# TUMFTM/global_racetrajectory_optimization

Measured on NVIDIA H100. Metric: min-curv QPs/sec (N=1000 closed track, batched), higher is better.
Workload: dtype f64

## Files before the change

global_racetrajectory_optimization_b200/csrc/mincurv_ipm.cu:

```cuda
#include <cstdio>
#include <cstdlib>
#include "capi.cuh"
#include "mincurv_ops.cuh"

namespace mc {

constexpr unsigned FULL = 0xffffffffu;
constexpr int IP_THREADS = 64;
constexpr int SUB = 8;
constexpr int VBP = 12;
constexpr int FROW = 33;
constexpr int HB_SLOTS = 2;
constexpr int HO_SLOTS = 2;
constexpr int LROW = 33;
#ifndef MC_LT_SLOTS
#define MC_LT_SLOTS 3
#endif
constexpr int LT_SLOTS = MC_LT_SLOTS;
constexpr int GT_SLOTS = 6 - LT_SLOTS;
constexpr int RING_UNITS = LT_SLOTS + GT_SLOTS;
constexpr int QDEPTH = 16;
constexpr int LT_UNIT_DOUBLES = SUB * LROW;
constexpr int GT_UNIT_DOUBLES = SUB * FROW;
constexpr unsigned HB_UNIT_BYTES = SUB * HB_PITCH * sizeof(double);
// ... 644 lines not shown
    sh.gs[lane] = gsl - (s0 + s1);
}

__device__ __noinline__ void sweep_sep_solve(IpShared &sh, double *__restrict__ GTp, const double *Zp, const int NA, double *__restrict__ x) {
    const int lane = threadIdx.x & 31;
    const int nunits = (NA + SUB - 1) / SUB;
    GtRing R(sh, &sh.u.sw.gt[0][0], GTp, nunits, true);
    R.prime();
    double a = sh.gs[lane];
#pragma unroll 4
    for (int k = 0; k < 32; ++k) {
        const double yk = __shfl_sync(FULL, a, k);
        const double l = (lane > k) ? sh.s.Ss[lane * 33 + k] : 0.0;
        a = fma(-l, yk, a);
    }
    a *= sh.wS[lane];
#pragma unroll 4
    for (int k = 31; k >= 0; --k) {
        const double xk = __shfl_sync(FULL, a, k);
        const double l = (lane < k) ? sh.s.Ss[k * 33 + lane] : 0.0;
        a = fma(-l, xk, a);
    }
    x[NA + lane] = a;
    const int kl = lane & 7, qr = lane >> 3;
    double xq[8];
#pragma unroll
    for (int i = 0; i < 8; ++i) xq[i] = __shfl_sync(FULL, a, 8 * qr + i);
    double znext = 0.0;
    if (nunits > 0 && R.unit(0) * SUB + kl < NA) znext = Zp[R.unit(0) * SUB + kl];
    for (int i = 0; i < nunits; ++i, R.next()) {
        const int k = R.unit(i) * SUB + kl;
        const double z = znext;
        if (i + 1 < nunits && R.unit(i + 1) * SUB + kl < NA) znext = Zp[R.unit(i + 1) * SUB + kl];
        if ((i & 7) == 0 && i >= 8) prog_wait<true>(sh, &sh.prog[2], i - 8);
        const double *gt = R.wait() + kl * FROW;
        double c0 = 0.0, c1 = 0.0;
#pragma unroll
        for (int e = 0; e < 8; e += 2) {
            c0 = fma(gt[8 * qr + e], xq[e], c0);
            c1 = fma(gt[8 * qr + e + 1], xq[e + 1], c1);
        }
        double c = c0 + c1;
        c += __shfl_xor_sync(FULL, c, 8);
        c += __shfl_xor_sync(FULL, c, 16);
        if (qr == 0) sh.u.sw.q[(i & (QDEPTH - 1)) * SUB + kl] = (k < NA) ? fma(-c, gt[32], z) : 0.0;
        __syncwarp();
        if (lane == 0) { prog_publish(&sh.prog[3], i + 1); R.refill(i); }
    }
    R.close();
}

__device__ __noinline__ void sweep_backward(IpShared &sh, double *__restrict__ LTp, const int NA, double *__restrict__ x) {
    const int lane = threadIdx.x & 31;
    const int gq = lane >> 2, q = lane & 3;
    const int nunits = (NA + SUB - 1) / SUB;
    LtRing R(sh, &sh.u.sw.lt[0][0], LTp, nunits, true);
    R.prime();
    double nbx[8];
#pragma unroll
    for (int i = 0; i < 8; ++i) nbx[i] = 0.0;
    for (int i = 0; i < nunits; ++i, R.next()) {
        const int k0 = R.unit(i) * SUB;
        const double *lt = R.wait();
        double a[10];
#pragma unroll
        for (int c = 0; c < 10; ++c) a[c] = lt_entry(lt, gq, 4 * c + q);
        double c0[2] = {0.0, 0.0}, c1[2] = {0.0, 0.0};
#pragma unroll
        for (int e = 2; e < 8; e += 2) {
            dmma(c0, a[2 + e], nbx[e]);
            dmma(c1, a[3 + e], nbx[e + 1]);
        }
        dmma(c0, a[2], nbx[0]);
        dmma(c1, a[3], nbx[1]);
        prog_wait(sh, &sh.prog[3], i + 1);
        const double t1 = sh.u.sw.q[(i & (QDEPTH - 1)) * SUB + gq];
        const double uu = t1 + (c0[0] + c1[0]);
        const double u0 = __shfl_sync(FULL, uu, 4 * q), u1 = __shfl_sync(FULL, uu, 16 + 4 * q);
        double d0[2] = {uu, uu}, d1[2] = {0.0, 0.0};
        dmma(d0, a[0], u0);
        dmma(d1, a[1], u1);
        const double x1 = d0[0] + d1[0];
        if (q == 0 && k0 + gq < NA) x[k0 + gq] = x1;
#pragma unroll
        for (int e = 7; e >= 2; --e) nbx[e] = nbx[e - 2];
        nbx[0] = -__shfl_sync(FULL, x1, 4 * q);
        nbx[1] = -__shfl_sync(FULL, x1, 16 + 4 * q);
        __syncwarp();
        if (lane == 0) { prog_publish(&sh.prog[2], i + 1); R.refill(i); }
    }
    R.close();
}

__device__ __noinline__ void solve(IpShared &sh, double *slab, const Layout &L, int n, const double *g, double *x, bool fused) {
    const Factor F = make_factor(slab, L, n, nullptr);
    const int warp = threadIdx.x >> 5;
    if (threadIdx.x < 4) sh.prog[threadIdx.x] = 0;
    fence_proxy_async();
    __syncthreads();
    if (!fused) {
        PROF_T0(t0);
        if (warp == 0) sweep_forward(sh, F.LT, F.Z, F.NA, g);
        else sweep_sep_rhs(sh, F.GT, F.NA, g);
        __syncthreads();
        PROF_ADD1(PROF_FWD_SWEEPS, t0);
    }
    PROF_T0(t3);
    if (warp == 1) sweep_sep_solve(sh, F.GT, F.Z, F.NA, x);
    else sweep_backward(sh, F.LT, F.NA, x);
    __syncthreads();
    PROF_ADD1(PROF_BWD_SWEEPS, t3);
}

__device__ void band_matvec(const double *__restrict__ HB, const double *__restrict__ v, double *__restrict__ out, int n) {
    for (int i = threadIdx.x; i < n; i += IP_THREADS) {
        const double *row = HB + (size_t)i * HB_PITCH;
        double s = row[0] * v[i];
        int j = i;
        for (int k = 1; k <= HBW; ++k) {
            j = (j + 1 == n) ? 0 : j + 1;
            s = fma(row[k], v[j], s);
        }
        j = i;
        for (int k = 1; k <= HBW; ++k) {
            j = (j == 0) ? n - 1 : j - 1;
            s = fma(HB[(size_t)j * HB_PITCH + k], v[j], s);
        }
        out[i] = s;
    }
}

__device__ __forceinline__ IpShared &ip_init_shared() {
    extern __shared__ __align__(16) unsigned char smem_raw[];
    IpShared &sh = *reinterpret_cast<IpShared *>(smem_raw);
    if (threadIdx.x == 0) {
        for (int i = 0; i < HB_SLOTS; ++i) mbar_init(&sh.hb_full[i], 1);
        for (int i = 0; i < HO_SLOTS; ++i) { mbar_init(&sh.ho_full[i], 1); mbar_init(&sh.ho_empty[i], 1); }
        for (int i = 0; i < RING_UNITS; ++i) mbar_init(&sh.ring_full[i], 1);
        sh.ring_phase[0] = 0; sh.ring_phase[1] = 0;
        asm volatile("fence.mbarrier_init.release.cluster;" ::: "memory");
    }
    __syncthreads();
    return sh;
}

__device__ __forceinline__ int next_instance(IpShared &sh, int *work_counter) {
    __syncthreads();
    if (threadIdx.x == 0) sh.next = atomicAdd(work_counter, 1);
    __syncthreads();
    return sh.next;
}

constexpr int V_PARK = V_VV;
enum ParkSlot {
    PARK_MU = 0, PARK_MU0 = 1, PARK_RDTOL = 2, PARK_IT = 3,
    PARK_TRACE = 8,
    PARK_MU_HIST = 16,
    PARK_LIST = 64
};
constexpr int PARK_BUCKETS = 24;
enum SchedSlot { SCHED_WORK = 0, SCHED_COUNT = 8, SCHED_TAKEN = 40 };
static_assert(SCHED_WORK < SCHED_COUNT && SCHED_COUNT + PARK_BUCKETS <= SCHED_TAKEN && SCHED_TAKEN + PARK_BUCKETS <= SCHED_INTS,
              "the schedule's counters behind the slabs");
static_assert(PARK_MU_HIST + 40 <= PARK_LIST && PARK_LIST + PARK_BUCKETS / 2 <= N_MIN + 64, "V_PARK slots within a vector");

__device__ __forceinline__ double *park_slots(double *ws, const Layout &L, int b) { return vec(ws + (size_t)b * L.stride, L, V_PARK); }
__device__ __forceinline__ int *park_list(double *ws, const Layout &L, int r) { return reinterpret_cast<int *>(park_slots(ws, L, r) + PARK_LIST); }
__device__ __forceinline__ int ld_relaxed(const int *p) {
    int v;
    asm volatile("ld.relaxed.gpu.global.s32 %0, [%1];" : "=r"(v) : "l"(p) : "memory");
    return v;
}

__device__ __forceinline__ int park_bucket(double mu, double mu_prev, double target, int left, int n, int n_max) {
    double r = left;
    if (mu <= target) r = 1.0;
    else if (mu < mu_prev) r = ceil(log(target / mu) / log(mu / mu_prev)) + 1.0;
    r = fmin(fmax(r, 1.0), (double)left);
    return min(PARK_BUCKETS - 1, (int)ceil(r * n / n_max));
}

__device__ __forceinline__ void park(int *sched, double *ws, const Layout &L, int b, int k) {
    __threadfence();
    const int r = atomicAdd(&sched[SCHED_COUNT + k], 1);
    atomicExch(&park_list(ws, L, r)[k], b + 1);
}

__device__ __forceinline__ int next_work(IpShared &sh, int *sched, double *ws, const Layout &L, int B) {
    __syncthreads();
    if (threadIdx.x == 0) {
        int b = B, resumed = 0;
        if (ld_relaxed(&sched[SCHED_WORK]) < B) b = atomicAdd(&sched[SCHED_WORK], 1);
        if (b >= B) {
            b = B;
            for (int k = PARK_BUCKETS - 1; k >= 0 && !resumed; --k) {
                int t = ld_relaxed(&sched[SCHED_TAKEN + k]);
                while (t < ld_relaxed(&sched[SCHED_COUNT + k])) {
                    const int seen = atomicCAS(&sched[SCHED_TAKEN + k], t, t + 1);
                    if (seen != t) { t = seen; continue; }
                    const int *e = &park_list(ws, L, t)[k];
                    int v = 0;
                    for (int spin = 0; spin < (1 << 24) && (v = ld_relaxed(e)) == 0; ++spin) __nanosleep(64);
                    __threadfence();
                    if (v > 0) { b = v - 1; resumed = 1; }
                    break;
                }
            }
        }
        sh.next = b;
        sh.resumed = resumed;
    }
    __syncthreads();
    return sh.next;
}

#ifdef MC_TAIL_TRACE
__device__ __forceinline__ double trace_clock() {
    unsigned long long t;
    asm volatile("mov.u64 %0, %%globaltimer;" : "=l"(t));
    return __longlong_as_double((long long)t);
}
#endif

template <bool ADD_ITERS>
__device__ __forceinline__ void write_instance(double *aout, int n, int n_max, const double *AL, int b, int result, int it,
                                               int32_t *status, int32_t *iters_out) {
    __syncthreads();
    for (int i = threadIdx.x; i < n_max; i += IP_THREADS) aout[i] = (i < n) ? AL[i] : 0.0;
    if (threadIdx.x == 0) {
        status[b] = result;
        if (iters_out) iters_out[b] = ADD_ITERS ? iters_out[b] + it : it;
    }
}

__device__ __forceinline__ double affine_step(double r) { return (r > 1.0) ? 1.0 / r : 1.0; }
__device__ __forceinline__ double centring(double c00, double c01, double c10, double c11, double ap, double ad, double mu, double m) {
    const double sigma = (c00 + ad * c01 + ap * c10 + ap * ad * c11) / m / mu;
    return sigma * sigma * sigma * mu;
}
__device__ __forceinline__ double damped_step(double eta, double r) { return (eta < r) ? eta / r : 1.0; }
__device__ __forceinline__ void corrector_terms(double smu, double su, double sl, double lu, double ll, double dx, double isu,
                                                double isl, double &tu, double &tl) {
    const double dlu = lu * (dx * isu - 1.0), dll = -ll * (1.0 + dx * isl);
    tu = smu - su * lu + dx * dlu;
    tl = smu - sl * ll - dx * dll;
}

__global__ void __launch_bounds__(IP_THREADS, 8)
mincurv_pdip_kernel(int B, int n_max, const int32_t *__restrict__ n_pts, double *__restrict__ ws, Layout L,
                    PdipParams prm, int slice, double *__restrict__ alpha_out, int32_t *__restrict__ status,
                    int32_t *__restrict__ iters_out, int *__restrict__ sched) {
#ifdef MC_DEBUG_SM_LIMIT
    {
        unsigned smid;
        asm volatile("mov.u32 %0, %%smid;" : "=r"(smid));
        if (smid >= MC_DEBUG_SM_LIMIT) return;
    }
#endif
    IpShared &sh = ip_init_shared();
    unsigned tick = 0;
    for (int b; (b = next_work(sh, sched, ws, L, B)) < B;) {
        const bool resume = sh.resumed;
        const int n = n_pts ? n_pts[b] : n_max;
        double *aout = alpha_out + (size_t)b * n_max;
        if (!resume && status[b] != 0) {
            for (int i = threadIdx.x; i < n_max; i += IP_THREADS) aout[i] = 0.0;
            if (iters_out && threadIdx.x == 0) iters_out[b] = 0;
            continue;
        }
        PROF_T0(tq0);
#ifdef MC_TAIL_TRACE
        if (threadIdx.x == 0) {
            double *PK = park_slots(ws, L, b);
            if (!resume) {
                unsigned smid;
                asm volatile("mov.u32 %0, %%smid;" : "=r"(smid));
                PK[PARK_TRACE + 2] = 0.0; PK[PARK_TRACE + 3] = 0.0; PK[PARK_TRACE + 5] = smid;
                PK[PARK_TRACE + 6] = 0.0; PK[PARK_TRACE + 7] = 0.0;
            }
            PK[PARK_TRACE + (resume ? 2 : 0)] = trace_clock();
        }
#endif
        double *slab = ws + (size_t)b * L.stride;
        const double *HB = ws + (size_t)*band_owner(slab, L) * L.stride + L.o_hb;
        const double *__restrict__ LB = vec(slab, L, V_LB), *__restrict__ UB = vec(slab, L, V_UB), *__restrict__ F = vec(slab, L, V_F);
        double *__restrict__ AL = vec(slab, L, V_ALPHA), *__restrict__ LU = vec(slab, L, V_LU), *__restrict__ LL = vec(slab, L, V_LL), *__restrict__ RD = vec(slab, L, V_RD);
        double *__restrict__ RHS = vec(slab, L, V_RHS), *__restrict__ DX = vec(slab, L, V_DX), *__restrict__ DXA = vec(slab, L, V_DXA);
        double *__restrict__ DD = vec(slab, L, V_DD), *__restrict__ SU = vec(slab, L, V_SU), *__restrict__ SL = vec(slab, L, V_SL);
        double *G0 = vec(slab, L, V_T0);
        if (threadIdx.x == 0) sh.flag = 0;
        double mu0, rd_tol, mu;
        int it;
        if (resume) {
            const double *PK = park_slots(ws, L, b);
            mu = PK[PARK_MU]; mu0 = PK[PARK_MU0]; rd_tol = PK[PARK_RDTOL]; it = (int)PK[PARK_IT];
        } else {
            for (int i = threadIdx.x; i < n; i += IP_THREADS) AL[i] = 0.5 * (LB[i] + UB[i]);
            __syncthreads();
            band_matvec(HB, AL, G0, n);
            __syncthreads();
            double gmax = 0.0, fmaxv = 0.0;
#pragma unroll 1
            for (int i = threadIdx.x; i < n; i += IP_THREADS) {
                const double gi = G0[i] + F[i];
                G0[i] = gi;
                gmax = fmax(gmax, fabs(gi));
                fmaxv = fmax(fmaxv, fabs(F[i]));
            }
            gmax = block_reduce<1>(gmax, sh.red);
            fmaxv = block_reduce<1>(fmaxv, sh.red);
            const double lam0 = prm.lam0_rel * gmax + 1e-300;
            double musum = 0.0;
#pragma unroll 1
            for (int i = threadIdx.x; i < n; i += IP_THREADS) {
                const double gi = G0[i];
                const double lu = fmax(-gi, 0.0) + lam0, ll = fmax(gi, 0.0) + lam0;
                const double rd = gi + lu - ll;
                LU[i] = lu; LL[i] = ll;
                RD[i] = rd;
                const double a = AL[i];
                const double su = UB[i] - a, sl = a - LB[i];
                const double isu = 1.0 / su, isl = 1.0 / sl;
                SU[i] = su; SL[i] = sl;
                DD[i] = lu * isu + ll * isl; RHS[i] = -rd + lu - ll;
                musum += su * lu + sl * ll;
            }
            musum = block_reduce<0>(musum, sh.red);
            mu0 = musum / (2.0 * n);
            rd_tol = prm.rd_rel * (fmaxv + gmax) + 1e-300;
            mu = mu0;
            it = 0;
        }
        int result = -1;
        const int it_end = (slice > 0 && !resume) ? min(slice, prm.max_iter) : prm.max_iter;

        constexpr int VG = 4, VS = VG * IP_THREADS;
        for (; it < it_end; ++it) {
            PROF_T0(tf0);
            const bool fok = factor(sh, slab, L, n, HB, RHS, tick);
            tick += factor_units(n);
            if (!fok) { result = 3; break; }
            PROF_ADD(PROF_FACTOR, tf0);
            PROF_T0(ts0);
            solve(sh, slab, L, n, RHS, DXA, true);
            PROF_ADD(PROF_SOLVE_PRED, ts0);
            PROF_T0(tv2);
            double rp = 0.0, rdl = 0.0, c00 = 0.0, c01 = 0.0, c10 = 0.0, c11 = 0.0;
#pragma unroll 1
            for (int i0 = threadIdx.x; i0 < n; i0 += VS) {
                double su[VG], sl[VG], lu[VG], ll[VG], dx[VG];
#pragma unroll
                for (int k = 0; k < VG; ++k) {
                    const int i = min(i0 + k * IP_THREADS, n - 1);
                    su[k] = SU[i]; sl[k] = SL[i]; lu[k] = LU[i]; ll[k] = LL[i]; dx[k] = DXA[i];
                }
#pragma unroll
                for (int k = 0; k < VG; ++k) {
                    if (i0 + k * IP_THREADS < n) {
                        const double isu = 1.0 / su[k], isl = 1.0 / sl[k];
                        const double p = dx[k] * isu, m = dx[k] * isl;
                        rp = fmax(rp, fmax(p, -m));
                        rdl = fmax(rdl, fmax(1.0 - p, 1.0 + m));
                        const double dlu = lu[k] * (p - 1.0), dll = -ll[k] * (1.0 + m);
                        c00 += su[k] * lu[k] + sl[k] * ll[k];
                        c01 += su[k] * dlu + sl[k] * dll;
                        c10 += dx[k] * (ll[k] - lu[k]);
                        c11 += dx[k] * (dll - dlu);
                    }
                }
            }
            rp = block_reduce<1>(rp, sh.red);
            rdl = block_reduce<1>(rdl, sh.red);
            double ap = affine_step(rp), ad = affine_step(rdl);
            c00 = block_reduce<0>(c00, sh.red); c01 = block_reduce<0>(c01, sh.red);
            c10 = block_reduce<0>(c10, sh.red); c11 = block_reduce<0>(c11, sh.red);
            const double smu = centring(c00, c01, c10, c11, ap, ad, mu, 2.0 * n);
            PROF_ADD(PROF_AFFINE, tv2);
            PROF_T0(tv3);
#pragma unroll 1
            for (int i0 = threadIdx.x; i0 < n; i0 += VS) {
                double su[VG], sl[VG], lu[VG], ll[VG], dx[VG], rd[VG];
#pragma unroll
                for (int k = 0; k < VG; ++k) {
                    const int i = min(i0 + k * IP_THREADS, n - 1);
                    su[k] = SU[i]; sl[k] = SL[i]; lu[k] = LU[i]; ll[k] = LL[i]; dx[k] = DXA[i]; rd[k] = RD[i];
                }
#pragma unroll
                for (int k = 0; k < VG; ++k) {
                    const int i = i0 + k * IP_THREADS;
                    if (i < n) {
                        const double isu = 1.0 / su[k], isl = 1.0 / sl[k];
                        double tu, tl;
                        corrector_terms(smu, su[k], sl[k], lu[k], ll[k], dx[k], isu, isl, tu, tl);
                        RHS[i] = -rd[k] - tu * isu + tl * isl;
                    }
                }
            }
            __syncthreads();
            PROF_ADD(PROF_CORR_RHS, tv3);
            PROF_T0(ts1);
            solve(sh, slab, L, n, RHS, DX, false);
            PROF_ADD(PROF_SOLVE_CORR, ts1);
            PROF_T0(tv4);
            rp = 0.0; rdl = 0.0;
#pragma unroll 1
            for (int i0 = threadIdx.x; i0 < n; i0 += VS) {
                double su[VG], sl[VG], lu[VG], ll[VG], dxa[VG], dx[VG];
#pragma unroll
                for (int k = 0; k < VG; ++k) {
                    const int i = min(i0 + k * IP_THREADS, n - 1);
                    su[k] = SU[i]; sl[k] = SL[i]; lu[k] = LU[i]; ll[k] = LL[i]; dxa[k] = DXA[i]; dx[k] = DX[i];
                }
#pragma unroll
                for (int k = 0; k < VG; ++k) {
                    if (i0 + k * IP_THREADS < n) {
                        const double isu = 1.0 / su[k], isl = 1.0 / sl[k];
                        double tu, tl;
                        corrector_terms(smu, su[k], sl[k], lu[k], ll[k], dxa[k], isu, isl, tu, tl);
                        const double dlu = (tu + lu[k] * dx[k]) * isu, dll = (tl - ll[k] * dx[k]) * isl;
                        rp = fmax(rp, fmax(dx[k] * isu, -dx[k] * isl));
                        rdl = fmax(rdl, fmax(-dlu / lu[k], -dll / ll[k]));
                    }
                }
            }
            rp = block_reduce<1>(rp, sh.red);
            rdl = block_reduce<1>(rdl, sh.red);
            ap = damped_step(prm.eta, rp);
            ad = damped_step(prm.eta, rdl);
            PROF_ADD(PROF_STEPLEN, tv4);
            PROF_T0(tv5);
            double musum2 = 0.0, rdmax = 0.0, dxmax = 0.0, amax = 0.0;
            constexpr int VG2 = 2, VS2 = VG2 * IP_THREADS;
#pragma unroll 1
            for (int i0 = threadIdx.x; i0 < n; i0 += VS2) {
                double su[VG2], sl[VG2], lu[VG2], ll[VG2], dxa[VG2], dx[VG2], al[VG2], rd[VG2], rh[VG2], dd[VG2];
#pragma unroll
                for (int k = 0; k < VG2; ++k) {
                    const int i = min(i0 + k * IP_THREADS, n - 1);
                    su[k] = SU[i]; sl[k] = SL[i]; lu[k] = LU[i]; ll[k] = LL[i]; dxa[k] = DXA[i]; dx[k] = DX[i];
                    al[k] = AL[i]; rd[k] = RD[i]; rh[k] = RHS[i]; dd[k] = DD[i];
                }
#pragma unroll
                for (int k = 0; k < VG2; ++k) {
                    const int i = i0 + k * IP_THREADS;
                    if (i < n) {
                        const double isu = 1.0 / su[k], isl = 1.0 / sl[k];
                        double tu, tl;
                        corrector_terms(smu, su[k], sl[k], lu[k], ll[k], dxa[k], isu, isl, tu, tl);
                        const double dlu = (tu + lu[k] * dx[k]) * isu, dll = (tl - ll[k] * dx[k]) * isl;
                        const double an = al[k] + ap * dx[k], lun = lu[k] + ad * dlu, lln = ll[k] + ad * dll;
                        const double sun = su[k] - ap * dx[k], sln = sl[k] + ap * dx[k];
                        const double rdn = rd[k] + ap * (rh[k] - dd[k] * dx[k]) + ad * (dlu - dll);
                        const double isun = 1.0 / sun, isln = 1.0 / sln;
                        AL[i] = an; LU[i] = lun; LL[i] = lln; RD[i] = rdn; SU[i] = sun; SL[i] = sln;
                        DD[i] = lun * isun + lln * isln; RHS[i] = -rdn + lun - lln;
                        musum2 += sun * lun + sln * lln;
                        rdmax = fmax(rdmax, fabs(rdn));
                        dxmax = fmax(dxmax, fabs(dx[k]));
                        amax = fmax(amax, fabs(an));
                    }
                }
            }
            if (threadIdx.x == 0) park_slots(ws, L, b)[PARK_MU] = mu;
            mu = block_reduce<0>(musum2, sh.red) / (2.0 * n);
            rdmax = block_reduce<1>(rdmax, sh.red);
            PROF_ADD(PROF_UPDATE, tv5);
#ifdef MC_TAIL_TRACE
            if (threadIdx.x == 0 && it < PARK_LIST - PARK_MU_HIST) {
                park_slots(ws, L, b)[PARK_MU_HIST + it] = mu;
                park_slots(ws, L, b)[PARK_MU0] = mu0;
            }
#endif
            bool settled = true;
            if (prm.dx_rel > 0.0 && mu <= prm.mu_rel * mu0) {
                dxmax = block_reduce<1>(dxmax, sh.red);
                amax = block_reduce<1>(amax, sh.red);
                settled = ap * dxmax <= prm.dx_rel * fmax(amax, 0.01);
            }
            if (mu <= prm.mu_rel * mu0 && rdmax <= rd_tol && settled) { result = 0; ++it; break; }
            if (mu <= 1e-4 * prm.mu_rel * mu0) { result = (rdmax <= 1e3 * rd_tol) ? 0 : 2; ++it; break; }
        }
        if (result < 0 && it < prm.max_iter) {
            if (threadIdx.x == 0) {
                double *PK = park_slots(ws, L, b);
                const double mu_prev = PK[PARK_MU];
                PK[PARK_MU] = mu; PK[PARK_MU0] = mu0; PK[PARK_RDTOL] = rd_tol; PK[PARK_IT] = it;
#ifdef MC_TAIL_TRACE
                PK[PARK_TRACE + 1] = trace_clock();
                PK[PARK_TRACE + 6] = it;
                PK[PARK_TRACE + 7] = park_bucket(mu, mu_prev, prm.mu_rel * mu0, prm.max_iter - it, n, n);
#endif
                park(sched, ws, L, b, park_bucket(mu, mu_prev, prm.mu_rel * mu0, prm.max_iter - it, n, n_max));
            }
            continue;
        }
        if (result < 0) result = 2;
        write_instance<false>(aout, n, n_max, AL, b, result, it, status, iters_out);
#ifdef MC_TAIL_TRACE
        if (threadIdx.x == 0) {
            double *PK = park_slots(ws, L, b);
            PK[PARK_TRACE + (resume ? 3 : 1)] = trace_clock();
            PK[PARK_TRACE + 4] = it;
        }
#endif
        PROF_ADD(PROF_TOTAL, tq0);
#ifdef MC_PROFILE
        if (blockIdx.x == 0 && threadIdx.x == 0) { atomicAdd(&g_prof[PROF_NQP], 1ull); atomicAdd(&g_prof[PROF_ITERS], (unsigned long long)it); }
#endif
    }
}

template <typename K>
static int ctas_per_sm(K kernel) {
    int nb = 0;
    if (cudaOccupancyMaxActiveBlocksPerMultiprocessor(&nb, kernel, IP_THREADS, sizeof(IpShared)) != cudaSuccess) return 1;
    return nb > 0 ? nb : 1;
}

struct SolverGrid {
    int grid;
    int *counter;
};
static SolverGrid solver_grid(int B, int n_max, void *workspace, int per_sm) {
    int dev = 0, sms = 132;
    cudaGetDevice(&dev);
    cudaDeviceGetAttribute(&sms, cudaDevAttrMultiProcessorCount, dev);
    int grid = sms * (per_sm > 0 ? per_sm : 1);
    if (grid > B) grid = B;
    return {grid, (int *)((char *)workspace + mincurv_slabs_bytes(B, n_max))};
}

template <typename... P, typename... A>
static int launch_solver(void (*kernel)(P...), int grid, int *work_counter, cudaStream_t stream, A... args) {
    cudaError_t e = cudaFuncSetAttribute(kernel, cudaFuncAttributeMaxDynamicSharedMemorySize, (int)sizeof(IpShared));
    if (e != cudaSuccess) return (int)e;
    if (work_counter) cudaMemsetAsync(work_counter, 0, sizeof(int), stream);
    kernel<<<grid, IP_THREADS, sizeof(IpShared), stream>>>(args...);
    return 0;
}

__global__ void __launch_bounds__(IP_THREADS, 8)
mincurv_pdip_kappa_kernel(int B, int n_max, const int32_t *__restrict__ n_pts, double *__restrict__ ws, Layout L,
                          PdipParams prm, double kb, double *__restrict__ alpha_out, int32_t *__restrict__ status,
                          int32_t *__restrict__ iters_out, int *__restrict__ work_counter) {
    IpShared &sh = ip_init_shared();
    unsigned tick = 0;
    for (int b; (b = next_instance(sh, work_counter)) < B;) {
        if (status[b] != 4) continue;
        const int n = n_pts ? n_pts[b] : n_max;
        double *aout = alpha_out + (size_t)b * n_max;
        double *slab = ws + (size_t)b * L.stride;
        const double *__restrict__ LB = vec(slab, L, V_LB), *__restrict__ UB = vec(slab, L, V_UB), *__restrict__ F = vec(slab, L, V_F);
        const double *__restrict__ KR = vec(slab, L, V_KREF);
        double *__restrict__ AL = vec(slab, L, V_ALPHA), *__restrict__ LU = vec(slab, L, V_LU), *__restrict__ LL = vec(slab, L, V_LL);
        double *__restrict__ RHS = vec(slab, L, V_RHS), *__restrict__ DX = vec(slab, L, V_DX), *__restrict__ DD = vec(slab, L, V_DD);
        double *__restrict__ TU = vec(slab, L, V_DLU), *__restrict__ TL = vec(slab, L, V_DLL), *__restrict__ SU = vec(slab, L, V_SU), *__restrict__ SL = vec(slab, L, V_SL);
        double *__restrict__ ISU = vec(slab, L, V_ISU), *__restrict__ ISL = vec(slab, L, V_ISL);
        double *__restrict__ S3 = vec(slab, L, V_S3), *__restrict__ S4 = vec(slab, L, V_S4), *__restrict__ L3 = vec(slab, L, V_L3), *__restrict__ L4 = vec(slab, L, V_L4);
        double *__restrict__ KL = vec(slab, L, V_KL), *__restrict__ WK = vec(slab, L, V_WK), *__restrict__ EDX = vec(slab, L, V_EDX);
        double *__restrict__ T3 = vec(slab, L, V_T3K), *__restrict__ T4 = vec(slab, L, V_T4K), *__restrict__ VV = vec(slab, L, V_VV), *__restrict__ ETV = vec(slab, L, V_RD);
        double *t0 = vec(slab, L, V_T0), *t1 = vec(slab, L, V_T1), *t2 = vec(slab, L, V_T2), *t3 = vec(slab, L, V_T3), *t4 = vec(slab, L, V_T4), *t5 = vec(slab, L, V_T5);
        const double m4 = 4.0 * n;
        if (threadIdx.x == 0) sh.flag = 0;

        for (int i = threadIdx.x; i < n; i += IP_THREADS) AL[i] = 0.5 * (LB[i] + UB[i]);
        __syncthreads();
        apply_E(slab, L, n, AL, EDX, t0, t1, t2, t3, t4, t5);
        apply_Et(slab, L, n, EDX, ETV, t0, t1, t2, t3, t4, t5);
        double gmax = 0.0, fmaxv = 0.0;
        for (int i = threadIdx.x; i < n; i += IP_THREADS) {
            gmax = fmax(gmax, fabs(ETV[i] + F[i]));
            fmaxv = fmax(fmaxv, fabs(F[i]));
        }
        gmax = block_reduce<1>(gmax, sh.red);
        fmaxv = block_reduce<1>(fmaxv, sh.red);
        const double lam0 = prm.lam0_rel * gmax + 1e-300;
        double musum = 0.0;
        for (int i = threadIdx.x; i < n; i += IP_THREADS) {
            const double gi = ETV[i] + F[i];
            const double lu = fmax(-gi, 0.0) + lam0, ll = fmax(gi, 0.0) + lam0;
            const double a = AL[i], su = UB[i] - a, sl = a - LB[i];
            const double kl = KR[i] + EDX[i];
            const double s3 = fmax(kb - kl, 1e-2 * kb), s4 = fmax(kb + kl, 1e-2 * kb);
            LU[i] = lu; LL[i] = ll; SU[i] = su; SL[i] = sl; ISU[i] = 1.0 / su; ISL[i] = 1.0 / sl;
            KL[i] = kl; S3[i] = s3; S4[i] = s4; L3[i] = lam0; L4[i] = lam0;
            musum += su * lu + sl * ll + (s3 + s4) * lam0;
        }
        musum = block_reduce<0>(musum, sh.red);
        const double mu0 = musum / m4;
        const double rd_tol = prm.rd_rel * (fmaxv + gmax) + 1e-300;
        double mu = mu0;
        int it = 0, result = 2;
        double rdmax = 1e300, rpmax = 1e300;
        for (it = 0; it < prm.max_iter + 20; ++it) {
            for (int i = threadIdx.x; i < n; i += IP_THREADS) {
                const double s3 = S3[i], s4 = S4[i], l3 = L3[i], l4 = L4[i], kl = KL[i];
                const double rp3 = kl + s3 - kb, rp4 = -kl + s4 - kb;
                WK[i] = l3 / s3 + l4 / s4;
                DD[i] = LU[i] * ISU[i] + LL[i] * ISL[i];
                VV[i] = (kl - KR[i]) + l3 * rp3 / s3 - l4 * rp4 / s4;
            }
            __syncthreads();
            assemble_hband(slab, L, n, WK, sh.u.win);
            __syncthreads();
            apply_Et(slab, L, n, VV, ETV, t0, t1, t2, t3, t4, t5);
            for (int i = threadIdx.x; i < n; i += IP_THREADS) RHS[i] = -F[i] - ETV[i];
            __syncthreads();
            const bool fok = factor(sh, slab, L, n, slab + L.o_hb, RHS, tick);
            tick += factor_units(n);
            if (!fok) {
                result = (mu <= 1e-7 * mu0 && rdmax <= 1e3 * rd_tol && rpmax <= 1e-6 * kb) ? 0 : 3;
                break;
            }
            solve(sh, slab, L, n, RHS, DX, true);
            apply_E(slab, L, n, DX, EDX, t0, t1, t2, t3, t4, t5);
            double rp = 0.0, rdl = 0.0, c00 = 0.0, c01 = 0.0, c10 = 0.0, c11 = 0.0;
            for (int i = threadIdx.x; i < n; i += IP_THREADS) {
                const double su = SU[i], sl = SL[i], lu = LU[i], ll = LL[i], dx = DX[i];
                const double s3 = S3[i], s4 = S4[i], l3 = L3[i], l4 = L4[i], kl = KL[i], ed = EDX[i];
                const double p = dx * ISU[i], m = dx * ISL[i];
                const double ds3 = -(kl + s3 - kb) - ed, ds4 = -(-kl + s4 - kb) + ed;
                const double dlu = lu * (p - 1.0), dll = -ll * (1.0 + m);
                const double dl3 = -l3 - l3 * ds3 / s3, dl4 = -l4 - l4 * ds4 / s4;
                rp = fmax(rp, fmax(fmax(p, -m), fmax(-ds3 / s3, -ds4 / s4)));
                rdl = fmax(rdl, fmax(fmax(1.0 - p, 1.0 + m), fmax(-dl3 / l3, -dl4 / l4)));
                c00 += su * lu + sl * ll + s3 * l3 + s4 * l4;
                c01 += su * dlu + sl * dll + s3 * dl3 + s4 * dl4;
                c10 += dx * (ll - lu) + ds3 * l3 + ds4 * l4;
                c11 += dx * (dll - dlu) + ds3 * dl3 + ds4 * dl4;
            }
            rp = block_reduce<1>(rp, sh.red);
            rdl = block_reduce<1>(rdl, sh.red);
            double ap = affine_step(rp), ad = affine_step(rdl);
            c00 = block_reduce<0>(c00, sh.red); c01 = block_reduce<0>(c01, sh.red);
            c10 = block_reduce<0>(c10, sh.red); c11 = block_reduce<0>(c11, sh.red);
            const double smu = centring(c00, c01, c10, c11, ap, ad, mu, m4);
            for (int i = threadIdx.x; i < n; i += IP_THREADS) {
                const double su = SU[i], sl = SL[i], lu = LU[i], ll = LL[i], dx = DX[i], isu = ISU[i], isl = ISL[i];
                const double s3 = S3[i], s4 = S4[i], l3 = L3[i], l4 = L4[i], kl = KL[i], ed = EDX[i];
                const double rp3 = kl + s3 - kb, rp4 = -kl + s4 - kb;
                const double ds3 = -rp3 - ed, ds4 = -rp4 + ed;
                const double dlu = lu * (dx * isu - 1.0), dll = -ll * (1.0 + dx * isl);
                const double dl3 = -l3 - l3 * ds3 / s3, dl4 = -l4 - l4 * ds4 / s4;
                const double tu = smu - su * lu + dx * dlu, tl = smu - sl * ll - dx * dll;
                const double q3 = smu - s3 * l3 - ds3 * dl3, q4 = smu - s4 * l4 - ds4 * dl4;
                TU[i] = tu; TL[i] = tl; T3[i] = q3; T4[i] = q4;
                VV[i] = (kl - KR[i]) + l3 - l4 + (q3 + l3 * rp3) / s3 - (q4 + l4 * rp4) / s4;
                RHS[i] = -(F[i] + lu - ll) - tu * isu + tl * isl;
            }
            __syncthreads();
            apply_Et(slab, L, n, VV, ETV, t0, t1, t2, t3, t4, t5);
            for (int i = threadIdx.x; i < n; i += IP_THREADS) RHS[i] -= ETV[i];
            __syncthreads();
            solve(sh, slab, L, n, RHS, DX, false);
            apply_E(slab, L, n, DX, EDX, t0, t1, t2, t3, t4, t5);
            rp = 0.0; rdl = 0.0;
            for (int i = threadIdx.x; i < n; i += IP_THREADS) {
                const double lu = LU[i], ll = LL[i], dx = DX[i], isu = ISU[i], isl = ISL[i];
                const double s3 = S3[i], s4 = S4[i], l3 = L3[i], l4 = L4[i], kl = KL[i], ed = EDX[i];
                const double ds3 = -(kl + s3 - kb) - ed, ds4 = -(-kl + s4 - kb) + ed;
                const double dlu = (TU[i] + lu * dx) * isu, dll = (TL[i] - ll * dx) * isl;
                const double dl3 = (T3[i] - l3 * ds3) / s3, dl4 = (T4[i] - l4 * ds4) / s4;
                rp = fmax(rp, fmax(fmax(dx * isu, -dx * isl), fmax(-ds3 / s3, -ds4 / s4)));
                rdl = fmax(rdl, fmax(fmax(-dlu / lu, -dll / ll), fmax(-dl3 / l3, -dl4 / l4)));
            }
            rp = block_reduce<1>(rp, sh.red);
            rdl = block_reduce<1>(rdl, sh.red);
            ap = damped_step(prm.eta, rp);
            ad = damped_step(prm.eta, rdl);
            double musum2 = 0.0;
            rpmax = 0.0;
            for (int i = threadIdx.x; i < n; i += IP_THREADS) {
                const double su = SU[i], sl = SL[i], lu = LU[i], ll = LL[i], dx = DX[i];
                const double s3 = S3[i], s4 = S4[i], l3 = L3[i], l4 = L4[i], kl = KL[i], ed = EDX[i];
                const double ds3 = -(kl + s3 - kb) - ed, ds4 = -(-kl + s4 - kb) + ed;
                const double dlu = (TU[i] + lu * dx) * ISU[i], dll = (TL[i] - ll * dx) * ISL[i];
                const double dl3 = (T3[i] - l3 * ds3) / s3, dl4 = (T4[i] - l4 * ds4) / s4;
                const double sun = su - ap * dx, sln = sl + ap * dx, s3n = s3 + ap * ds3, s4n = s4 + ap * ds4;
                const double lun = lu + ad * dlu, lln = ll + ad * dll, l3n = l3 + ad * dl3, l4n = l4 + ad * dl4;
                const double kln = kl + ap * ed;
                AL[i] += ap * dx; SU[i] = sun; SL[i] = sln; ISU[i] = 1.0 / sun; ISL[i] = 1.0 / sln;
                LU[i] = lun; LL[i] = lln; S3[i] = s3n; S4[i] = s4n; L3[i] = l3n; L4[i] = l4n; KL[i] = kln;
                VV[i] = (kln - KR[i]) + l3n - l4n;
                musum2 += sun * lun + sln * lln + s3n * l3n + s4n * l4n;
                rpmax = fmax(rpmax, fmax(fabs(kln + s3n - kb), fabs(-kln + s4n - kb)));
            }
            mu = block_reduce<0>(musum2, sh.red) / m4;
            rpmax = block_reduce<1>(rpmax, sh.red);
            __syncthreads();
            apply_Et(slab, L, n, VV, ETV, t0, t1, t2, t3, t4, t5);
            rdmax = 0.0;
            for (int i = threadIdx.x; i < n; i += IP_THREADS) rdmax = fmax(rdmax, fabs(ETV[i] + F[i] + LU[i] - LL[i]));
            rdmax = block_reduce<1>(rdmax, sh.red);
            if (mu <= prm.mu_rel * mu0 && rdmax <= rd_tol && rpmax <= 1e-8 * kb) { result = 0; ++it; break; }
            if (mu <= 1e-2 * prm.mu_rel * mu0) { result = (rdmax <= 1e3 * rd_tol && rpmax <= 1e-6 * kb) ? 0 : 2; ++it; break; }
        }
        write_instance<true>(aout, n, n_max, AL, b, result, it, status, iters_out);
    }
}

__global__ void __launch_bounds__(IP_THREADS, 8)
debug_factor_solve_kernel(int B, int n_max, const int32_t *__restrict__ n_pts, double *__restrict__ ws, Layout L,
                          int32_t *__restrict__ status) {
    IpShared &sh = ip_init_shared();
    unsigned tick = 0;
    for (int b = blockIdx.x; b < B; b += gridDim.x) {
        const int n = n_pts ? n_pts[b] : n_max;
        double *slab = ws + (size_t)b * L.stride;
        if (threadIdx.x == 0) sh.flag = 0;
        __syncthreads();
        const bool ok = factor(sh, slab, L, n, slab + L.o_hb, vec(slab, L, V_RHS), tick);
        tick += factor_units(n);
        solve(sh, slab, L, n, vec(slab, L, V_RHS), vec(slab, L, V_DX), true);
        solve(sh, slab, L, n, vec(slab, L, V_T0), vec(slab, L, V_T1), false);
        const bool ok2 = factor(sh, slab, L, n, slab + L.o_hb, vec(slab, L, V_T0), tick);
        tick += factor_units(n);
        solve(sh, slab, L, n, vec(slab, L, V_T0), vec(slab, L, V_T2), true);
        if (threadIdx.x == 0) status[b] = (ok && ok2) ? 0 : 3;
        __syncthreads();
    }
}

__global__ void __launch_bounds__(IP_THREADS, 8)
mincurv_adjoint_kernel(int B, int n_max, const int32_t *__restrict__ n_pts, const double *__restrict__ reftrack, double w_veh,
                       const double *__restrict__ w_veh_batch, double *__restrict__ ws, Layout L, const double *__restrict__ sens,
                       const double *__restrict__ grad_alpha, int32_t *__restrict__ grad_status,
                       double *__restrict__ grad_w_right, double *__restrict__ grad_w_left, double *__restrict__ grad_w_veh,
                       int *__restrict__ work_counter) {
    IpShared &sh = ip_init_shared();
    unsigned tick = 0;
    for (int b; (b = next_instance(sh, work_counter)) < B;) {
        const int n = n_pts ? n_pts[b] : n_max;
        double *gwr = grad_w_right + (size_t)b * n_max, *gwl = grad_w_left + (size_t)b * n_max;
        bool ok = grad_status[b] == 0;
        if (ok) {
            double *slab = ws + (size_t)b * L.stride;
            const double *HB = ws + (size_t)*band_owner(slab, L) * L.stride + L.o_hb;
            const double *__restrict__ DU = sens + (size_t)b * 2 * n_max, *__restrict__ DL = DU + n_max;
            const double *__restrict__ GA = grad_alpha + (size_t)b * n_max;
            double *__restrict__ RHS = vec(slab, L, V_RHS), *__restrict__ DX = vec(slab, L, V_DX), *__restrict__ DD = vec(slab, L, V_DD);
            if (threadIdx.x == 0) sh.flag = 0;
            for (int i = threadIdx.x; i < L.np; i += IP_THREADS) {
                if (i < n) DD[i] = DU[i] + DL[i];
                RHS[i] = (i < n) ? GA[i] : 0.0;
            }
            ok = factor(sh, slab, L, n, HB, RHS, tick);
            tick += factor_units(n);
            if (ok) {
                solve(sh, slab, L, n, RHS, DX, true);
                const double wv = w_veh_batch ? w_veh_batch[b] : w_veh;
                const double *rt = reftrack + (size_t)b * n_max * 4;
                double gv = 0.0;
                for (int i = threadIdx.x; i < n_max; i += IP_THREADS) {
                    double gr = 0.0, gl = 0.0;
                    if (i < n) {
                        const double v = DX[i], gu = DU[i] * v, glb = DL[i] * v;
                        const double2 ww = *reinterpret_cast<const double2 *>(rt + (size_t)i * 4 + 2);
                        const double ub = ww.x - 0.5 * wv, lb = -(ww.y - 0.5 * wv);
                        if (ub - lb < 2.0 * FIX_EPS) {
                            gr = 0.5 * (gu + glb);
                            gl = -gr;
                        } else {
                            gr = gu;
                            gl = -glb;
                            gv += 0.5 * (glb - gu);
                        }
                    }
                    gwr[i] = gr;
                    gwl[i] = gl;
                }
                gv = block_reduce<0>(gv, sh.red);
                if (threadIdx.x == 0) grad_w_veh[b] = gv;
                continue;
            }
            if (threadIdx.x == 0) grad_status[b] = 3;
        }
        for (int i = threadIdx.x; i < n_max; i += IP_THREADS) { gwr[i] = 0.0; gwl[i] = 0.0; }
        if (threadIdx.x == 0) grad_w_veh[b] = 0.0;
    }
}

}

static constexpr int PDIP_SLICE_DEFAULT = 8;

extern "C" {

int mc_mincurv_pdip_batch(int B, int n_max, const int32_t *n_pts, double *alpha, int32_t *status, int32_t *iters,
                          void *workspace, size_t workspace_bytes, void *stream) {
    if (!alpha || !status) return bad("mc_mincurv_pdip_batch: NULL argument");
    int rc = mc::mincurv_args("mc_mincurv_pdip_batch", B, n_max, workspace, workspace_bytes);
    if (rc) return rc;
    mc::PdipParams prm;
    prm.max_iter = 40;
    prm.mu_rel = 1e-10;
    prm.rd_rel = 1e-8;
    prm.eta = 0.995;
    prm.dx_rel = 1e-5;
    prm.lam0_rel = 1e-2;
    if (const char *e = getenv("MC_DEBUG_PDIP_LAM0")) { const double v = atof(e); if (v > 0.0) prm.lam0_rel = v; }
    if (const char *e = getenv("MC_DEBUG_PDIP_ETA")) { const double v = atof(e); if (v > 0.5 && v < 1.0) prm.eta = v; }
    if (const char *e = getenv("MC_DEBUG_PDIP_DX_REL")) { const double v = atof(e); if (v >= 0.0) prm.dx_rel = v; }
    if (const char *e = getenv("MC_DEBUG_PDIP_MU_REL")) { const double v = atof(e); if (v > 0.0) prm.mu_rel = v; }
    int per_sm = mc::ctas_per_sm(mc::mincurv_pdip_kernel);
    if (const char *e = getenv("MC_DEBUG_PDIP_CTAS_PER_SM")) {
        const int v = atoi(e);
        if (v > 0 && v < per_sm) per_sm = v;
    }
    int slice = PDIP_SLICE_DEFAULT;
    if (const char *e = getenv("MC_DEBUG_PDIP_SLICE")) { const int v = atoi(e); if (v >= 0) slice = v; }
    const mc::SolverGrid g = mc::solver_grid(B, n_max, workspace, per_sm);
    const mc::Layout L = mc::make_layout(n_max);
    double *ws = (double *)workspace;
    cudaStream_t s = (cudaStream_t)stream;
    if (B <= g.grid) slice = 0;
    cudaMemsetAsync(g.counter, 0, mc::SCHED_INTS * sizeof(int), s);
    if (slice > 0)
        cudaMemset2DAsync(ws + (size_t)mc::V_PARK * L.np + mc::PARK_LIST, L.stride * sizeof(double), 0,
                          mc::PARK_BUCKETS * sizeof(int), B, s);
    if (mc::launch_solver(mc::mincurv_pdip_kernel, g.grid, nullptr, s, B, n_max, n_pts, ws, L, prm, slice, alpha, status, iters,
                          g.counter) != 0) {
        snprintf(mc::g_err, sizeof(mc::g_err), "mincurv_pdip_kernel: cudaFuncSetAttribute failed");
        return MC_ECUDA;
    }
    return check_cuda("mincurv_pdip_kernel");
}

int mc_mincurv_kappa_batch(int B, int n_max, const int32_t *n_pts, double kappa_bound, double *alpha, int32_t *status,
                           int32_t *iters, void *workspace, size_t workspace_bytes, void *stream) {
    if (!alpha || !status) return bad("mc_mincurv_kappa_batch: NULL argument");
    int rc = mc::mincurv_args("mc_mincurv_kappa_batch", B, n_max, workspace, workspace_bytes);
    if (rc) return rc;
    mc::PdipParams prm;
    prm.max_iter = 40;
    prm.mu_rel = 1e-11;
    prm.rd_rel = 1e-8;
    prm.eta = 0.995;
    prm.dx_rel = 0.0;
    prm.lam0_rel = 1e-2;
    const mc::SolverGrid g = mc::solver_grid(B, n_max, workspace, mc::ctas_per_sm(mc::mincurv_pdip_kappa_kernel));
    if (mc::launch_solver(mc::mincurv_pdip_kappa_kernel, g.grid, g.counter, (cudaStream_t)stream, B, n_max, n_pts,
                          (double *)workspace, mc::make_layout(n_max), prm, kappa_bound, alpha, status, iters, g.counter) != 0) {
        snprintf(mc::g_err, sizeof(mc::g_err), "mincurv_pdip_kappa_kernel: cudaFuncSetAttribute failed");
        return MC_ECUDA;
    }
    return check_cuda("mincurv_pdip_kappa_kernel");
}

int mc_mincurv_adjoint_batch(int B, int n_max, const int32_t *n_pts, const double *reftrack, const double *normvec,
                             const double *h, double w_veh, const double *w_veh_batch, double f_scale, const int32_t *centre_id,
                             const double *sens, int32_t *grad_status, const double *grad_alpha, double *grad_w_right,
                             double *grad_w_left, double *grad_w_veh, void *workspace, size_t workspace_bytes, void *stream) {
    if (!sens || !grad_status || !grad_alpha || !grad_w_right || !grad_w_left || !grad_w_veh)
        return bad("mc_mincurv_adjoint_batch: NULL argument");
    int rc = mc_mincurv_setup_batch_shared(B, n_max, n_pts, reftrack, normvec, h, w_veh, w_veh_batch, f_scale, centre_id,
                                           reinterpret_cast<int32_t *>(grad_w_right), workspace, workspace_bytes, stream);
    if (rc) return rc;
    const mc::SolverGrid g = mc::solver_grid(B, n_max, workspace, mc::ctas_per_sm(mc::mincurv_adjoint_kernel));
    if (mc::launch_solver(mc::mincurv_adjoint_kernel, g.grid, g.counter, (cudaStream_t)stream, B, n_max, n_pts, reftrack, w_veh,
                          w_veh_batch, (double *)workspace, mc::make_layout(n_max), sens, grad_alpha, grad_status, grad_w_right,
                          grad_w_left, grad_w_veh, g.counter) != 0) {
        snprintf(mc::g_err, sizeof(mc::g_err), "mincurv_adjoint_kernel: cudaFuncSetAttribute failed");
        return MC_ECUDA;
    }
    return check_cuda("mincurv_adjoint_kernel");
}

int mc_debug_factor_solve(int B, int n_max, const int32_t *n_pts, int32_t *status, void *workspace, size_t workspace_bytes,
                          void *stream) {
    if (!status) return bad("mc_debug_factor_solve: NULL argument");
    int rc = mc::mincurv_args("mc_debug_factor_solve", B, n_max, workspace, workspace_bytes);
    if (rc) return rc;
    const mc::SolverGrid g = mc::solver_grid(B, n_max, workspace, mc::ctas_per_sm(mc::debug_factor_solve_kernel));
    if (mc::launch_solver(mc::debug_factor_solve_kernel, g.grid, nullptr, (cudaStream_t)stream, B, n_max, n_pts,
                          (double *)workspace, mc::make_layout(n_max), status) != 0)
        return bad("mc_debug_factor_solve: cudaFuncSetAttribute failed");
    return check_cuda("debug_factor_solve_kernel");
}

int mc_debug_read_profile(unsigned long long *host_out24, int reset) {
#ifdef MC_PROFILE
    if (cudaMemcpyFromSymbol(host_out24, mc::g_prof, sizeof(unsigned long long) * mc::PROF_SLOTS) != cudaSuccess) return MC_ECUDA;
    if (getenv("MC_PROFILE_SEGMENTS")) {
        unsigned long long seg[32];
        if (cudaMemcpyFromSymbol(seg, mc::g_seg, sizeof(seg)) == cudaSuccess) {
            fprintf(stderr, "segments:");
            for (int i = 0; i < 32; ++i) fprintf(stderr, " %d:%llu", i, seg[i]);
            fprintf(stderr, "\n");
        }
    }
    if (reset) {
        unsigned long long z[32] = {0};
        if (cudaMemcpyToSymbol(mc::g_prof, z, sizeof(unsigned long long) * mc::PROF_SLOTS) != cudaSuccess) return MC_ECUDA;
        cudaMemcpyToSymbol(mc::g_seg, z, sizeof(z));
    }
    return MC_OK;
#else
    (void)reset;
    for (int i = 0; i < mc::PROF_SLOTS; ++i) host_out24[i] = 0ull;
    return MC_OK;
#endif
}

}
```

Measured before the change: 70080.

## Allow repeated parking of QP instances with reslicing and warp-parallel bucket scan

The persistent solver could previously park a QP instance only once, after its first slice. Instances can now be re-parked up to a budget of times, resuming in short reslices and running to completion once the predicted remaining iterations fit in one reslice. The park list is extended to hold several entries per bucket per instance, and next_work scans all buckets in parallel with a warp ballot instead of a serial loop by thread 0. Default slice sizes are reduced. The aim is to balance the tail of the batch by letting long-running instances be redistributed more finely, at the cost of extra park/resume overhead and more global atomics.

Result: no change. 71020, median of 6 (+1.3%).

```diff
diff --git a/global_racetrajectory_optimization_b200/csrc/mincurv_ipm.cu b/global_racetrajectory_optimization_b200/csrc/mincurv_ipm.cu
--- a/global_racetrajectory_optimization_b200/csrc/mincurv_ipm.cu
+++ b/global_racetrajectory_optimization_b200/csrc/mincurv_ipm.cu
@@ -820,63 +820,78 @@
 }
 
 constexpr int V_PARK = V_VV;
+constexpr int PARK_BUCKETS = 24;
+constexpr int PARK_BUDGET = 5;
 enum ParkSlot {
-    PARK_MU = 0, PARK_MU0 = 1, PARK_RDTOL = 2, PARK_IT = 3,
-    PARK_TRACE = 8,
-    PARK_MU_HIST = 16,
-    PARK_LIST = 64
+    PARK_MU = 0, PARK_MU0 = 1, PARK_RDTOL = 2, PARK_IT = 3, PARK_PARKS = 4,
+    PARK_MU_HIST = 8,
+    PARK_LIST = 48,
+    PARK_TRACE = PARK_LIST + PARK_BUDGET * PARK_BUCKETS / 2,
+    PARK_END = PARK_TRACE + 4 * (PARK_BUDGET + 1)
 };
-constexpr int PARK_BUCKETS = 24;
 enum SchedSlot { SCHED_WORK = 0, SCHED_COUNT = 8, SCHED_TAKEN = 40 };
 static_assert(SCHED_WORK < SCHED_COUNT && SCHED_COUNT + PARK_BUCKETS <= SCHED_TAKEN && SCHED_TAKEN + PARK_BUCKETS <= SCHED_INTS,
               "the schedule's counters behind the slabs");
-static_assert(PARK_MU_HIST + 40 <= PARK_LIST && PARK_LIST + PARK_BUCKETS / 2 <= N_MIN + 64, "V_PARK slots within a vector");
+static_assert(PARK_BUCKETS <= 32, "one lane of a warp per bucket (next_work)");
+static_assert(PARK_PARKS < PARK_MU_HIST && PARK_MU_HIST + 40 <= PARK_LIST && PARK_END <= N_MIN + 64, "V_PARK slots within a vector");
 
 __device__ __forceinline__ double *park_slots(double *ws, const Layout &L, int b) { return vec(ws + (size_t)b * L.stride, L, V_PARK); }
-__device__ __forceinline__ int *park_list(double *ws, const Layout &L, int r) { return reinterpret_cast<int *>(park_slots(ws, L, r) + PARK_LIST); }
+__device__ __forceinline__ int *park_entry(double *ws, const Layout &L, int B, int k, int t) {
+    return reinterpret_cast<int *>(park_slots(ws, L, t % B) + PARK_LIST) + (t / B) * PARK_BUCKETS + k;
+}
 __device__ __forceinline__ int ld_relaxed(const int *p) {
     int v;
     asm volatile("ld.relaxed.gpu.global.s32 %0, [%1];" : "=r"(v) : "l"(p) : "memory");
     return v;
 }
 
-__device__ __forceinline__ int park_bucket(double mu, double mu_prev, double target, int left, int n, int n_max) {
+__device__ __forceinline__ double predicted_remaining(double mu, double mu_prev, double target, int left) {
     double r = left;
     if (mu <= target) r = 1.0;
     else if (mu < mu_prev) r = ceil(log(target / mu) / log(mu / mu_prev)) + 1.0;
-    r = fmin(fmax(r, 1.0), (double)left);
-    return min(PARK_BUCKETS - 1, (int)ceil(r * n / n_max));
-}
-
-__device__ __forceinline__ void park(int *sched, double *ws, const Layout &L, int b, int k) {
+    return fmin(fmax(r, 1.0), (double)left);
+}
+
+__device__ __forceinline__ void park(int *sched, double *ws, const Layout &L, int B, int b, double r, int n, int n_max) {
+    const int k = min(PARK_BUCKETS - 1, (int)ceil(r * n / n_max));
     __threadfence();
-    const int r = atomicAdd(&sched[SCHED_COUNT + k], 1);
-    atomicExch(&park_list(ws, L, r)[k], b + 1);
+    const int t = atomicAdd(&sched[SCHED_COUNT + k], 1);
+    atomicExch(park_entry(ws, L, B, k, t), b + 1);
 }
 
 __device__ __forceinline__ int next_work(IpShared &sh, int *sched, double *ws, const Layout &L, int B) {
     __syncthreads();
-    if (threadIdx.x == 0) {
-        int b = B, resumed = 0;
-        if (ld_relaxed(&sched[SCHED_WORK]) < B) b = atomicAdd(&sched[SCHED_WORK], 1);
+    if (threadIdx.x < 32) {
+        const unsigned FULL = 0xffffffffu;
+        const int lane = threadIdx.x;
+        int b = B;
+        if (lane == 0 && ld_relaxed(&sched[SCHED_WORK]) < B) b = atomicAdd(&sched[SCHED_WORK], 1);
+        b = __shfl_sync(FULL, b, 0);
+        int resumed = 0;
         if (b >= B) {
             b = B;
-            for (int k = PARK_BUCKETS - 1; k >= 0 && !resumed; --k) {
-                int t = ld_relaxed(&sched[SCHED_TAKEN + k]);
-                while (t < ld_relaxed(&sched[SCHED_COUNT + k])) {
-                    const int seen = atomicCAS(&sched[SCHED_TAKEN + k], t, t + 1);
-                    if (seen != t) { t = seen; continue; }
-                    const int *e = &park_list(ws, L, t)[k];
-                    int v = 0;
+            for (;;) {
+                int t = 0, c = 0;
+                if (lane < PARK_BUCKETS) {
+                    t = ld_relaxed(&sched[SCHED_TAKEN + lane]);
+                    c = ld_relaxed(&sched[SCHED_COUNT + lane]);
+                }
+                const unsigned open = __ballot_sync(FULL, t < c);
+                if (open == 0) break;
+                const int k = 31 - __clz(open);
+                int v = 0;
+                if (lane == k && atomicCAS(&sched[SCHED_TAKEN + k], t, t + 1) == t) {
+                    const int *e = park_entry(ws, L, B, k, t);
                     for (int spin = 0; spin < (1 << 24) && (v = ld_relaxed(e)) == 0; ++spin) __nanosleep(64);
                     __threadfence();
-                    if (v > 0) { b = v - 1; resumed = 1; }
-                    break;
+                    if (v == 0) v = -1;
                 }
-            }
-        }
-        sh.next = b;
-        sh.resumed = resumed;
+                v = __shfl_sync(FULL, v, k);
+                if (v > 0) { b = v - 1; resumed = 1; }
+                if (v != 0) break;
+            }
+        }
+        if (lane == 0) { sh.next = b; sh.resumed = resumed; }
     }
     __syncthreads();
     return sh.next;
@@ -916,7 +931,7 @@
 
 __global__ void __launch_bounds__(IP_THREADS, 8)
 mincurv_pdip_kernel(int B, int n_max, const int32_t *__restrict__ n_pts, double *__restrict__ ws, Layout L,
-                    PdipParams prm, int slice, double *__restrict__ alpha_out, int32_t *__restrict__ status,
+                    PdipParams prm, int slice, int reslice, double *__restrict__ alpha_out, int32_t *__restrict__ status,
                     int32_t *__restrict__ iters_out, int *__restrict__ sched) {
 #ifdef MC_DEBUG_SM_LIMIT
     {
@@ -940,13 +955,11 @@
 #ifdef MC_TAIL_TRACE
         if (threadIdx.x == 0) {
             double *PK = park_slots(ws, L, b);
-            if (!resume) {
-                unsigned smid;
-                asm volatile("mov.u32 %0, %%smid;" : "=r"(smid));
-                PK[PARK_TRACE + 2] = 0.0; PK[PARK_TRACE + 3] = 0.0; PK[PARK_TRACE + 5] = smid;
-                PK[PARK_TRACE + 6] = 0.0; PK[PARK_TRACE + 7] = 0.0;
-            }
-            PK[PARK_TRACE + (resume ? 2 : 0)] = trace_clock();
+            if (!resume)
+                for (int i = PARK_TRACE; i < PARK_END; ++i) PK[i] = 0.0;
+            double *part = PK + PARK_TRACE + 4 * (resume ? (int)PK[PARK_PARKS] : 0);
+            part[0] = trace_clock();
+            part[3] = blockIdx.x;
         }
 #endif
         double *slab = ws + (size_t)b * L.stride;
@@ -958,10 +971,11 @@
         double *G0 = vec(slab, L, V_T0);
         if (threadIdx.x == 0) sh.flag = 0;
         double mu0, rd_tol, mu;
-        int it;
+        int it, it_end;
         if (resume) {
             const double *PK = park_slots(ws, L, b);
             mu = PK[PARK_MU]; mu0 = PK[PARK_MU0]; rd_tol = PK[PARK_RDTOL]; it = (int)PK[PARK_IT];
+            it_end = ((int)PK[PARK_PARKS] < PARK_BUDGET) ? min(it + reslice, prm.max_iter) : prm.max_iter;
         } else {
             for (int i = threadIdx.x; i < n; i += IP_THREADS) AL[i] = 0.5 * (LB[i] + UB[i]);
             __syncthreads();
@@ -998,11 +1012,13 @@
             rd_tol = prm.rd_rel * (fmaxv + gmax) + 1e-300;
             mu = mu0;
             it = 0;
+            it_end = (slice > 0) ? min(slice, prm.max_iter) : prm.max_iter;
+            if (threadIdx.x == 0) park_slots(ws, L, b)[PARK_PARKS] = 0.0;
         }
         int result = -1;
-        const int it_end = (slice > 0 && !resume) ? min(slice, prm.max_iter) : prm.max_iter;
 
         constexpr int VG = 4, VS = VG * IP_THREADS;
+    next_slice:
         for (; it < it_end; ++it) {
             PROF_T0(tf0);
             const bool fok = factor(sh, slab, L, n, HB, RHS, tick);
@@ -1149,16 +1165,18 @@
             if (mu <= 1e-4 * prm.mu_rel * mu0) { result = (rdmax <= 1e3 * rd_tol) ? 0 : 2; ++it; break; }
         }
         if (result < 0 && it < prm.max_iter) {
+            const double remaining = predicted_remaining(mu, park_slots(ws, L, b)[PARK_MU], prm.mu_rel * mu0, prm.max_iter - it);
+            if (resume && remaining <= reslice) { it_end = prm.max_iter; goto next_slice; }
+            __syncthreads();
             if (threadIdx.x == 0) {
                 double *PK = park_slots(ws, L, b);
-                const double mu_prev = PK[PARK_MU];
-                PK[PARK_MU] = mu; PK[PARK_MU0] = mu0; PK[PARK_RDTOL] = rd_tol; PK[PARK_IT] = it;
+                const int parks = (int)PK[PARK_PARKS];
+                PK[PARK_MU] = mu; PK[PARK_MU0] = mu0; PK[PARK_RDTOL] = rd_tol; PK[PARK_IT] = it; PK[PARK_PARKS] = parks + 1;
 #ifdef MC_TAIL_TRACE
-                PK[PARK_TRACE + 1] = trace_clock();
-                PK[PARK_TRACE + 6] = it;
-                PK[PARK_TRACE + 7] = park_bucket(mu, mu_prev, prm.mu_rel * mu0, prm.max_iter - it, n, n);
-#endif
-                park(sched, ws, L, b, park_bucket(mu, mu_prev, prm.mu_rel * mu0, prm.max_iter - it, n, n_max));
+                PK[PARK_TRACE + 4 * parks + 1] = trace_clock();
+                PK[PARK_TRACE + 4 * parks + 2] = it;
+#endif
+                park(sched, ws, L, B, b, remaining, n, n_max);
             }
             continue;
         }
@@ -1167,8 +1185,9 @@
 #ifdef MC_TAIL_TRACE
         if (threadIdx.x == 0) {
             double *PK = park_slots(ws, L, b);
-            PK[PARK_TRACE + (resume ? 3 : 1)] = trace_clock();
-            PK[PARK_TRACE + 4] = it;
+            const int parks = (int)PK[PARK_PARKS];
+            PK[PARK_TRACE + 4 * parks + 1] = trace_clock();
+            PK[PARK_TRACE + 4 * parks + 2] = it;
         }
 #endif
         PROF_ADD(PROF_TOTAL, tq0);
@@ -1450,7 +1469,8 @@
 
 }
 
-static constexpr int PDIP_SLICE_DEFAULT = 8;
+static constexpr int PDIP_SLICE_DEFAULT = 6;
+static constexpr int PDIP_RESLICE_DEFAULT = 3;
 
 extern "C" {
 
@@ -1475,8 +1495,13 @@
         const int v = atoi(e);
         if (v > 0 && v < per_sm) per_sm = v;
     }
-    int slice = PDIP_SLICE_DEFAULT;
-    if (const char *e = getenv("MC_DEBUG_PDIP_SLICE")) { const int v = atoi(e); if (v >= 0) slice = v; }
+    int slice = PDIP_SLICE_DEFAULT, reslice = PDIP_RESLICE_DEFAULT;
+    if (const char *e = getenv("MC_DEBUG_PDIP_SLICE")) {
+        char *end = nullptr;
+        const long v = strtol(e, &end, 10);
+        if (v >= 0) slice = (int)v;
+        if (*end == ',') { const long v2 = strtol(end + 1, nullptr, 10); if (v2 > 0) reslice = (int)v2; }
+    }
     const mc::SolverGrid g = mc::solver_grid(B, n_max, workspace, per_sm);
     const mc::Layout L = mc::make_layout(n_max);
     double *ws = (double *)workspace;
@@ -1485,9 +1510,9 @@
     cudaMemsetAsync(g.counter, 0, mc::SCHED_INTS * sizeof(int), s);
     if (slice > 0)
         cudaMemset2DAsync(ws + (size_t)mc::V_PARK * L.np + mc::PARK_LIST, L.stride * sizeof(double), 0,
-                          mc::PARK_BUCKETS * sizeof(int), B, s);
-    if (mc::launch_solver(mc::mincurv_pdip_kernel, g.grid, nullptr, s, B, n_max, n_pts, ws, L, prm, slice, alpha, status, iters,
-                          g.counter) != 0) {
+                          mc::PARK_BUDGET * mc::PARK_BUCKETS * sizeof(int), B, s);
+    if (mc::launch_solver(mc::mincurv_pdip_kernel, g.grid, nullptr, s, B, n_max, n_pts, ws, L, prm, slice, reslice, alpha, status,
+                          iters, g.counter) != 0) {
         snprintf(mc::g_err, sizeof(mc::g_err), "mincurv_pdip_kernel: cudaFuncSetAttribute failed");
         return MC_ECUDA;
     }
```
